# piyanon108/iGate4xSoftphoneDSP

Hardware: AMD Instinct MI355X
Metric: Msamples/s G.711 decode+RMS, 65536ch@8kHz; %HBM roofline at 1/2/4/8 GPU (higher is better)
Workload: dtype u8

## Files before the change

### igate4xsoftphonedsp_amd/csrc/igdsp_device.h

```cpp
#pragma once
#include "igdsp_internal.h"

#include <algorithm>
#include <cstdlib>

namespace igdsp {

__device__ __forceinline__ uint32_t ulaw_abs(uint32_t code)
{
    const uint32_t u = ~code & 0x7Fu;
    return ((((u & 15u) * 2u + 33u) << (u >> 4)) - 33u) << 2;
}

__device__ __forceinline__ uint32_t alaw_abs(uint32_t code)
{
    const uint32_t a = (code ^ 0x55u) & 0x7Fu;
    const uint32_t s = a >> 4, q = a & 15u;
    const uint32_t m = (s == 0u) ? (q * 2u + 1u) : ((q * 2u + 33u) << (s - 1u));
    return m << 3;
}

typedef uint32_t u32x4_t __attribute__((ext_vector_type(4)));
__device__ __forceinline__ uint4 ld_stream(const uint4 *p)
{
// ... 28 lines not shown
__device__ __forceinline__ __amdgpu_buffer_rsrc_t make_rsrc_ranged(const void *base, uint32_t bytes)
{
    return __builtin_amdgcn_make_buffer_rsrc(const_cast<void *>(base), 0, (int)bytes, 0x00020000);
}
__device__ __forceinline__ uint4 buf_ld_stream(__amdgpu_buffer_rsrc_t r, uint32_t voff, uint32_t soff)
{
    const u32x4_t v = __builtin_amdgcn_raw_buffer_load_b128(r, (int)voff, (int)soff, 2);
    return make_uint4(v.x, v.y, v.z, v.w);
}
#ifndef IGDSP_RTS_LOAD_AUX
#define IGDSP_RTS_LOAD_AUX 2
#endif
__device__ __forceinline__ uint4 buf_ld_pieces(__amdgpu_buffer_rsrc_t r, uint32_t voff, uint32_t soff)
{
    const u32x4_t v = __builtin_amdgcn_raw_buffer_load_b128(r, (int)voff, (int)soff, IGDSP_RTS_LOAD_AUX);
    return make_uint4(v.x, v.y, v.z, v.w);
}
__device__ __forceinline__ void buf_st(__amdgpu_buffer_rsrc_t r, uint32_t voff, uint32_t soff, const uint4 v)
{
    u32x4_t t; t.x = v.x; t.y = v.y; t.z = v.z; t.w = v.w;
    __builtin_amdgcn_raw_buffer_store_b128(t, r, (int)voff, (int)soff, 0);
}

#ifndef IGDSP_RECORD_STORE
#define IGDSP_RECORD_STORE 2
#endif
__device__ __forceinline__ void st_record_block(igdsp_frame_stats *base, uint32_t lane, const uint4 v)
{
#if IGDSP_RECORD_STORE == 2
    u32x4_t t; t.x = v.x; t.y = v.y; t.z = v.z; t.w = v.w;
    __builtin_amdgcn_raw_buffer_store_b128(t, make_rsrc(base), (int)(lane * 16u), 0, 16);
#elif IGDSP_RECORD_STORE == 1
    u32x4_t t; t.x = v.x; t.y = v.y; t.z = v.z; t.w = v.w;
    __builtin_nontemporal_store(t, reinterpret_cast<u32x4_t *>(base) + lane);
#else
    st_stream(reinterpret_cast<uint4 *>(base) + lane, v);
#endif
}

__device__ __forceinline__ uint32_t full_scale(bool alaw) { return alaw ? 32256u : 32124u; }

__device__ __forceinline__ uint64_t shfl_xor_u64(uint64_t v, int m)
{
    uint32_t lo = (uint32_t)v, hi = (uint32_t)(v >> 32);
    lo = (uint32_t)__shfl_xor((int)lo, m, 64);
    hi = (uint32_t)__shfl_xor((int)hi, m, 64);
    return ((uint64_t)hi << 32) | lo;
}

__device__ __forceinline__ void agg_commit_block(igdsp_aggregate *agg, uint32_t rank, uint2 *slots, uint32_t nwaves,
                                                 uint64_t sumsq, uint64_t samples, uint32_t frames, uint32_t n_silent,
                                                 uint32_t n_clipped, uint32_t bm_sum, uint32_t peak)
{
    const uint32_t lane = threadIdx.x & 63u, wave = threadIdx.x >> 6;
#pragma unroll
    for (int m = 32; m >= 1; m >>= 1) {
        sumsq += shfl_xor_u64(sumsq, m);
        samples += shfl_xor_u64(samples, m);
        frames += (uint32_t)__shfl_xor((int)frames, m, 64);
        n_silent += (uint32_t)__shfl_xor((int)n_silent, m, 64);
// ... 259 lines not shown
    for (int j = 0; j < kLoadsPerChunk; ++j) {
        const uint32_t p = (uint32_t)j * 64u + lane, f = p / 10u, q = p - f * 10u;
        const uint32_t sh = q == 1u ? 0u : (q == 3u ? 8u : (q == 2u ? 16u : 24u));
        fr5 |= f << (5 * j);
        pm5 |= sh << (5 * j);
    }
}

#ifndef IGDSP_SPREAD_METER
#define IGDSP_SPREAD_METER 0
#endif
__device__ __forceinline__ uint32_t spread_batch(uint32_t b, uint32_t nb)
{
#ifdef IGDSP_NO_SPREAD
    return b;
#endif
    const uint32_t half = (nb + 1u) >> 1;
    return b >= nb ? b : ((b & 1u) ? half + (b >> 1) : (b >> 1));
}

template <int W>
struct BlockQueue { uint32_t next, batch[8], tag[8]; };

template <int W>
__device__ __forceinline__ void bq_init(BlockQueue<W> &q, uint32_t *gq, uint32_t G, uint32_t gb1)
{
    q.next = (uint32_t)W;
    for (int i = 0; i < 8; ++i) q.tag[i] = 0xFFFFFFFFu;
    q.batch[0] = blockIdx.x; q.tag[0] = 0u;
    q.batch[1] = gq ? gb1 + G : blockIdx.x + G; q.tag[1] = 1u;
}

template <int W>
__device__ __forceinline__ uint32_t bq_grab(BlockQueue<W> &q, uint32_t *gq, uint32_t G, uint32_t lane, uint32_t nb)
{
    uint32_t v = 0;
    if (lane == 0) {
        const uint32_t s = atomicAdd(&q.next, 1u);
        const uint32_t j = s / (uint32_t)W, w = s - j * (uint32_t)W;
        if (w == 0u) {
            const uint32_t nb = gq ? atomicAdd(gq, 1u) + G : blockIdx.x + (j + 1u) * G;
            __hip_atomic_store(&q.batch[(j + 1u) & 7u], nb, __ATOMIC_RELAXED, __HIP_MEMORY_SCOPE_WORKGROUP);
            __hip_atomic_store(&q.tag[(j + 1u) & 7u], j + 1u, __ATOMIC_RELEASE, __HIP_MEMORY_SCOPE_WORKGROUP);
        }
        while (__hip_atomic_load(&q.tag[j & 7u], __ATOMIC_ACQUIRE, __HIP_MEMORY_SCOPE_WORKGROUP) != j)
            __builtin_amdgcn_s_sleep(2);
        v = spread_batch(__hip_atomic_load(&q.batch[j & 7u], __ATOMIC_RELAXED, __HIP_MEMORY_SCOPE_WORKGROUP), nb) * (uint32_t)W + w;
    }
    return (uint32_t)__builtin_amdgcn_readfirstlane((int)v);
}

__device__ __forceinline__ void bq_finish(uint32_t *gq, uint32_t G)
{
    if (gq == nullptr) return;
    __syncthreads();
    if (threadIdx.x == 0 && atomicAdd(gq + 1, 1u) == G - 1u) { gq[0] = 0u; gq[1] = 0u; }
}

template <typename T> __device__ __forceinline__ void lds_add(T *p, T v) { __hip_atomic_fetch_add(p, v, __ATOMIC_RELAXED, __HIP_MEMORY_SCOPE_WORKGROUP); }
__device__ __forceinline__ void lds_max(uint32_t *p, uint32_t v) { __hip_atomic_fetch_max(p, v, __ATOMIC_RELAXED, __HIP_MEMORY_SCOPE_WORKGROUP); }
__device__ __forceinline__ void lds_min(uint32_t *p, uint32_t v) { __hip_atomic_fetch_min(p, v, __ATOMIC_RELAXED, __HIP_MEMORY_SCOPE_WORKGROUP); }
__device__ __forceinline__ uint32_t wave_draw(uint32_t *counter, uint32_t lane)
{
    uint32_t v = 0;
// ... 181 lines not shown
```

### igate4xsoftphonedsp_amd/csrc/igdsp_k_meter.hip

```cpp
#include "igdsp_device.h"

namespace igdsp {

__global__ __launch_bounds__(256) void k_meter_wave_per_frame(
    const uint8_t *__restrict__ payload, const uint8_t *__restrict__ codec, const uint16_t *__restrict__ len,
    uint32_t C, uint32_t first_frame, uint32_t n_frames, uint32_t n, igdsp_frame_stats *__restrict__ stats,
    int16_t *__restrict__ pcm, igdsp_aggregate *agg, uint32_t rank)
{
    __shared__ int16_t lut[2][256];
    __shared__ uint2 agg_slots[4 * 4];
    for (uint32_t i = threadIdx.x; i < 512u; i += 256u) {
        const uint32_t code = i & 255u;
        const int ax = (int)((i >> 8) ? alaw_abs(code) : ulaw_abs(code));
        lut[i >> 8][code] = (int16_t)((code & 0x80u) ? ax : -ax);
    }
    __syncthreads();

    const uint32_t lane = threadIdx.x & 63u, wave = threadIdx.x >> 6;
    const bool dword_ok = ((n & 3u) == 0u) && ((reinterpret_cast<uintptr_t>(payload) & 3u) == 0u) &&
                          ((reinterpret_cast<uintptr_t>(pcm) & 7u) == 0u);
    uint64_t a_sumsq = 0, a_samples = 0;
    uint32_t a_frames = 0, a_sil = 0, a_clip = 0, a_bm = 0, a_peak = 0;

    auto load_frame = [&](uint32_t fi) -> uint32_t {
// ... 376 lines not shown
                        u_sil += (uint32_t)__builtin_popcountll(__ballot((fl & IGDSP_FLAG_SILENT) != 0u));
                        u_clip += (uint32_t)__builtin_popcountll(__ballot((fl & IGDSP_FLAG_CLIPPED) != 0u));
                    }
                }
                wave_lds_fence();
            }
            if (done) break;
        }
    }
    if (AGG && agg != nullptr) {
        const bool l0 = lane == 0u;
        agg_commit_block(agg, rank, lds + kLutEntries, (uint32_t)kFatWaves, a_sumsq, l0 ? (uint64_t)u_frames * kFrame : 0ull, l0 ? u_frames : 0u,
                         l0 ? u_sil : 0u, l0 ? u_clip : 0u, a_bm, a_peak);
    }
}

constexpr int kImgMaxPieces = IGDSP_MAX_PAYLOAD * kSuperFrames / 16 / 64;

template <bool AGG, bool RAGGED>
__global__ __launch_bounds__(kImgMaxWaves * 64) void k_meter_image(
    const uint8_t *__restrict__ payload, const uint8_t *__restrict__ codec, const uint16_t *__restrict__ len, uint32_t C,
    uint32_t first_frame, uint32_t n_frames, uint32_t n, igdsp_frame_stats *__restrict__ stats, igdsp_aggregate *agg, uint32_t rank)
{
    __shared__ uint2 lut[kLutEntries];
    extern __shared__ __attribute__((aligned(16))) uint8_t img_smem[];
    const uint32_t n_waves = blockDim.x >> 6;
    fill_lut(lut);
    __syncthreads();
    const uint32_t lane = threadIdx.x & 63u, wave = (uint32_t)__builtin_amdgcn_readfirstlane((int)(threadIdx.x >> 6));
    const uint32_t img_bytes = (uint32_t)kSuperFrames * n;
    uint32_t *img = reinterpret_cast<uint32_t *>(img_smem + (size_t)wave * img_bytes);
    const uint32_t off = (lane & 31u) * 8u;
    const uint32_t D = n >> 2;
    const uint32_t np = (img_bytes / 16u + 63u) >> 6;
    const uint32_t n_items = (n_frames - first_frame + (uint32_t)kSuperFrames - 1u) / (uint32_t)kSuperFrames;
    const uint64_t total_bytes = (uint64_t)n_frames * n;
    const uint8_t *base0 = payload + (uint64_t)first_frame * n;

    uint64_t a_sumsq = 0;
    uint32_t a_samp = 0, a_bm = 0, a_peak = 0;
    uint32_t u_frames = 0, u_sil = 0, u_clip = 0;

    uint4 d[kImgMaxPieces];
    auto avail_of = [&](uint32_t it) {
        const uint64_t b = (uint64_t)first_frame * n + (uint64_t)it * img_bytes;
        return (uint32_t)min((uint64_t)img_bytes, total_bytes - b);
    };
    auto fetch = [&](uint32_t it) {
        const uint8_t *src = base0 + (uint64_t)it * img_bytes;
        const uint32_t avail = avail_of(it);
// ... 81 lines not shown
                    uint32_t w = row[i];
                    const uint32_t nv = min(l - 4u * i, 4u);
                    const uint32_t t = (w & 0x7F7F7F7Fu) | lm;
                    const uint2 e0 = lut_at(lut, t, off, 0x0C0C0400u), e1 = lut_at(lut, t, off, 0x0C0C0500u);
                    const uint2 e2 = lut_at(lut, t, off, 0x0C0C0600u), e3 = lut_at(lut, t, off, 0x0C0C0700u);
                    if (nv == 4u) {
                        part += e0.x + e1.x + e2.x + e3.x;
                        peak = max(max(peak, e0.y), max(e1.y, max(e2.y, e3.y)));
                    } else {
                        part += e0.x + (nv > 1u ? e1.x : 0u) + (nv > 2u ? e2.x : 0u);
                        peak = max(max(peak, e0.y), max(nv > 1u ? e1.y : 0u, nv > 2u ? e2.y : 0u));
                        w &= (1u << (8u * nv)) - 1u;
                    }
                    bsum = __builtin_amdgcn_sad_u8(w, 0u, bsum);
                }
            }
            s += part;
        }
        bool probe = false;
        if (l > 48u) probe = ((row[7] & 0xFFu) == 0xD5u) && (((row[9] >> 16) & 0xFFu) == 0xD5u) && ((row[12] & 0xFFu) == 0xD5u);
        uint32_t bm = 0, fl = 0;
        uint4 rec = make_uint4(0u, 0u, 0u, (uint32_t)IGDSP_FLAG_EMPTY << 24);
        if (l != 0u) rec = pack_stats(s << 4, peak, bsum, l, alaw, probe, bm, fl);
        if (live) st_stream(reinterpret_cast<uint4 *>(stats + fi), rec);
        if (AGG) {
            const bool met = l != 0u;
            if (met) { a_sumsq += s << 4; a_samp += l; a_bm += bm; a_peak = max(a_peak, peak); }
            u_frames += (uint32_t)__builtin_popcountll(__ballot(met));
            u_sil += (uint32_t)__builtin_popcountll(__ballot(met && (fl & IGDSP_FLAG_SILENT) != 0u));
            u_clip += (uint32_t)__builtin_popcountll(__ballot(met && (fl & IGDSP_FLAG_CLIPPED) != 0u));
        }
        wave_lds_fence();
    }
    if (AGG && agg != nullptr) {
        __shared__ uint2 agg_slots[kWavesPerBlock * 4];
        const bool l0 = lane == 0u;
        agg_commit_block(agg, rank, agg_slots, n_waves, a_sumsq, (uint64_t)a_samp, l0 ? u_frames : 0u, l0 ? u_sil : 0u, l0 ? u_clip : 0u, a_bm, a_peak);
    }
}


template <int Q, bool TAIL, bool AGG, bool STORE = false>
__global__ __launch_bounds__((StridedGeom<Q + (TAIL ? 1 : 0), STORE>::kWaves * 64)) void k_meter_strided(
    const uint8_t *__restrict__ payload, const uint8_t *__restrict__ codec, uint32_t C, uint32_t n_frames, uint32_t n,
    igdsp_frame_stats *__restrict__ stats, igdsp_aggregate *agg, uint32_t rank, uint32_t *gqueue, int16_t *__restrict__ pcm = nullptr)
{
    static_assert(Q == 1 || Q >= 4, "the probe bytes 28 / 38 / 48 are taken from pieces 1 / 2 / 3");
    constexpr int QP = Q + (TAIL ? 1 : 0);
    constexpr int kWaves = StridedGeom<QP, STORE>::kWaves;
    constexpr int kRow = QP | 1;
    constexpr int kStrip = kSuperFrames * kRow;
    constexpr int kLutU2 = STORE ? kLutEntries : kLut32Words / 2;
    __shared__ uint2 lds[kLutU2 + kWaves * kStrip + (STORE ? kWaves * 256 : 0)];
    __shared__ BlockQueue<kWaves> bq;
    __shared__ AggBlock aggb;
    uint32_t gb1 = 0;
    if (threadIdx.x == 0 && gqueue != nullptr) gb1 = atomicAdd(gqueue, 1u);
    if (STORE) fill_lut(lds); else fill_lut32(reinterpret_cast<uint32_t *>(lds));
    if (threadIdx.x == 0) { bq_init(bq, gqueue, gridDim.x, gb1); agg_block_init(aggb); }
    __syncthreads();

    const uint32_t lane = threadIdx.x & 63u, wave = (uint32_t)__builtin_amdgcn_readfirstlane((int)(threadIdx.x >> 6));
    uint2 *strip = lds + kLutU2 + wave * kStrip;
    uint8_t *xpose = STORE ? reinterpret_cast<uint8_t *>(lds + kLutU2 + kWaves * kStrip + wave * 256) : nullptr;
    const uint32_t off = (lane & 31u) * (STORE ? 8u : 4u);
    const uint32_t *l32 = reinterpret_cast<const uint32_t *>(lds);
    const uint32_t T = (n - 16u * Q) >> 2;
    constexpr int kPk = (QP + 1) / 2;
    constexpr bool kPoRegs = !STORE || QP <= 11;
    uint32_t pk[kPk];
    uint32_t po[kPoRegs ? QP : 1];
#pragma unroll
    for (int j = 0; j < kPk; ++j) pk[j] = 0;
#pragma unroll
    for (int j = 0; j < QP; ++j) {
        const uint32_t p = (uint32_t)j * 64u + lane, f = p / (uint32_t)QP, q = p - f * (uint32_t)QP;
        const uint32_t sh = q == 1u ? 0u : (q == 3u ? 8u : (q == 2u ? 16u : 24u));
        const bool tp = TAIL && q == (uint32_t)Q;
        pk[j >> 1] |= ((f << 2) | ((tp ? 24u : sh) << 8) | (tp ? 0x2000u : 0u)) << (16 * (j & 1));
        if (kPoRegs) po[j] = f * n + (tp ? n - 16u : 16u * q);
    }
// ... 145 lines not shown
#pragma unroll
                    for (int t = 0; t < 2; ++t)
                        if ((uint32_t)t < T) {
                            const uint32_t w = tws[t];
                            if (STORE) {
                                const uint32_t tt = (w & 0x7F7F7F7Fu) | lm;
                                const uint2 e0 = lut_at(lds, tt, off, 0x0C0C0400u), e1 = lut_at(lds, tt, off, 0x0C0C0500u);
                                const uint2 e2 = lut_at(lds, tt, off, 0x0C0C0600u), e3 = lut_at(lds, tt, off, 0x0C0C0700u);
                                s += (uint64_t)(e0.x + e1.x + e2.x + e3.x);
                                peak = max(max(peak, e0.y), max(e1.y, max(e2.y, e3.y)));
                            } else {
                                const uint32_t ot = off | (lm & 0x80u);
                                const uint32_t q0 = lut32_at(l32, w, ot, 0x0C0C0400u), q1 = lut32_at(l32, w, ot, 0x0C0C0500u);
                                const uint32_t q2 = lut32_at(l32, w, ot, 0x0C0C0600u), q3 = lut32_at(l32, w, ot, 0x0C0C0700u);
                                s += (uint64_t)(q0 + q1 + q2 + q3);
                                tail_m2 = max(tail_m2, max(max(q0, q1), max(q2, q3)));
                            }
                            bsum = __builtin_amdgcn_sad_u8(w, 0u, bsum);
                        }
                    if (!STORE) peak = max(peak, isqrt_m2(tail_m2) << 2);
                }
                const bool probe = (Q >= 4) && (fail >> 31) == 0u;
                uint32_t bm, fl;
                st_stream(reinterpret_cast<uint4 *>(stats + (f0 + lane)), pack_stats(s << 4, peak, bsum, n, my_alaw, probe, bm, fl));
                if (AGG) {
                    a_sumsq += s << 4; a_bm += bm; a_peak = max(a_peak, peak);
                    u_frames += (uint32_t)kSuperFrames;
                    u_sil += (uint32_t)__builtin_popcountll(__ballot((fl & IGDSP_FLAG_SILENT) != 0u));
                    u_clip += (uint32_t)__builtin_popcountll(__ballot((fl & IGDSP_FLAG_CLIPPED) != 0u));
                }
            }
            wave_lds_fence();
            return nxt_pt;
        };
        auto load_item = [&](uint4 (&d)[QP], const uint32_t s) __attribute__((always_inline)) {
            const uint8_t *b0 = payload + (uint64_t)s * item_bytes;
#pragma unroll
            for (int j = 0; j < QP; ++j) d[j] = ld16_dw(b0 + po_of(j));
        };
        if (!kTwoAhead) {
            uint4 d[QP];
            uint32_t sidx = sidx0, cur_pt = fetch_pt(sidx);
            load_item(d, sidx);
            uint32_t s_next = grab();
            for (;;) {
                const bool has_next = s_next < n_super;
                uint32_t s_after;
// ... 88 lines not shown
    for (int d = 0; d < kTinyDepth; ++d) { ids[d] = next_item(); fetch(ids[d], q[d]); }
#endif
    auto step = [&](Item &slot, uint32_t &id) __attribute__((always_inline)) -> bool {
        const uint32_t it = id;
        if (it == 0xFFFFFFFFu) return false;
        const Item x = slot;
        id = next_item();
        fetch(id, slot);
        const bool alaw = x.pt == IGDSP_PT_PCMA;
        const uint32_t oj = off | (alaw ? 0x80u : 0u);
        uint32_t sum = 0, mx = 0, bsum = 0;
        auto dword = [&](uint32_t w) {
            const uint32_t q0 = lut32_at(l32, w, oj, 0x0C0C0400u), q1 = lut32_at(l32, w, oj, 0x0C0C0500u);
            const uint32_t q2 = lut32_at(l32, w, oj, 0x0C0C0600u), q3 = lut32_at(l32, w, oj, 0x0C0C0700u);
            sum = sum + q0 + q1; sum = sum + q2 + q3;
            mx = max(max(mx, q0), q1); mx = max(max(mx, q2), q3);
            bsum = __builtin_amdgcn_sad_u8(w, 0u, bsum);
        };
        dword(x.a.x); dword(x.a.y); dword(x.a.z); dword(x.a.w);
#pragma unroll
        for (int k = 4; k < N4; ++k) dword(x.b[k - 4]);
        const uint32_t peak = isqrt_m2(mx) << 2;
        uint32_t bm, fl;
        st_stream(reinterpret_cast<uint4 *>(stats + ((uint64_t)it * (uint32_t)kSuperFrames + lane)),
                  pack_stats((uint64_t)sum << 4, peak, bsum, n, alaw, false, bm, fl));
        if (AGG) {
            a_sumsq += (uint64_t)sum << 4; a_bm += bm; a_peak = max(a_peak, peak);
            u_frames += (uint32_t)kSuperFrames;
            u_sil += (uint32_t)__builtin_popcountll(__ballot((fl & IGDSP_FLAG_SILENT) != 0u));
            u_clip += (uint32_t)__builtin_popcountll(__ballot((fl & IGDSP_FLAG_CLIPPED) != 0u));
        }
        return true;
    };
    static_assert(kTinyDepth == 4, "the loop below names the four register sets");
    while (step(q[0], ids[0]) && step(q[1], ids[1]) && step(q[2], ids[2]) && step(q[3], ids[3])) {}
    wave_exit(AGG ? agg : nullptr, rank, aggb, (uint32_t)kTinyWaves, lane, gqueue, G, a_sumsq, lane == 0u ? (uint64_t)u_frames * n : 0ull,
              a_bm, a_peak, u_frames, u_sil, u_clip);
}

hipError_t init_device_attributes()
{
    const int lim = 160 * 1024 - 2048 - kLutEntries * 8;
    const void *fns[] = {reinterpret_cast<const void *>(&k_meter_image<true, true>), reinterpret_cast<const void *>(&k_meter_image<false, true>),
                         reinterpret_cast<const void *>(&k_meter_image<true, false>), reinterpret_cast<const void *>(&k_meter_image<false, false>)};
    for (const void *f : fns) {
        const hipError_t e = hipFuncSetAttribute(f, hipFuncAttributeMaxDynamicSharedMemorySize, lim);
        if (e != hipSuccess) return e;
    }
// ... 59 lines not shown
```

### igate4xsoftphonedsp_amd/csrc/igdsp_k_packets.hip

```cpp
#include "igdsp_device.h"
#include "igdsp_rtp.h"

namespace igdsp {

constexpr int kSlotPieces = IGDSP_SLOT_BYTES / 16;
constexpr int kRtpHalfLoads = kSlotPieces * kChunkFrames / 64;
constexpr int kRtpRow = kSlotPieces + 2;
constexpr int kRtpStrip = kSuperFrames * kRtpRow;

template <bool SLOT, bool MIXED = false>
__device__ __forceinline__ void rtp_half(const uint2 *lut, uint2 *strip_half, uint4 (&d)[kRtpHalfLoads],
                                         const uint32_t am, const uint32_t (&fr)[kRtpHalfLoads], const uint32_t (&pm)[kRtpHalfLoads],
                                         const uint32_t off, const uint32_t lane,
                                         const uint8_t *refill_base, const uint32_t (&roff)[kRtpHalfLoads], const uint32_t nrm = 0u)
{
    uint2 e[2][8];
    uint32_t wa[2], wb[2];
    auto issue = [&](int u) {
        const int j = u >> 1, k = u & 1;
        wa[k] = (u & 1) ? d[j].z : d[j].x;
        wb[k] = (u & 1) ? d[j].w : d[j].y;
        const uint32_t lmj = (uint32_t)__builtin_amdgcn_sbfe(am, fr[j], 1) & 0x80808080u;
        const uint32_t ta = (wa[k] & 0x7F7F7F7Fu) | lmj, tb = (wb[k] & 0x7F7F7F7Fu) | lmj;
        e[k][0] = lut_at(lut, ta, off, 0x0C0C0400u); e[k][1] = lut_at(lut, ta, off, 0x0C0C0500u);
        e[k][2] = lut_at(lut, ta, off, 0x0C0C0600u); e[k][3] = lut_at(lut, ta, off, 0x0C0C0700u);
        e[k][4] = lut_at(lut, tb, off, 0x0C0C0400u); e[k][5] = lut_at(lut, tb, off, 0x0C0C0500u);
        e[k][6] = lut_at(lut, tb, off, 0x0C0C0600u); e[k][7] = lut_at(lut, tb, off, 0x0C0C0700u);
// ... 113 lines not shown
    }
}

template <bool AGG, bool SLOT, bool MIXED = false, int WIN = 0>
__global__ __launch_bounds__(kRtpWaves * 64) void k_meter_rtp64(
    const uint8_t *__restrict__ slots, const uint16_t *__restrict__ sizes, const uint8_t *__restrict__ codec, uint32_t C,
    uint32_t n_frames, uint32_t stride, uint32_t hdr, igdsp_frame_stats *__restrict__ stats, igdsp_rtp_info *__restrict__ info,
    igdsp_aggregate *agg, uint32_t rank, uint32_t *gqueue, const uint8_t *__restrict__ radio = nullptr, const WinArgs win = WinArgs{})
{
    static_assert(!(SLOT && MIXED), "slots always hold 20-byte headers");
    if (MIXED) hdr = 12u;
    __shared__ __attribute__((aligned(16))) uint2 lds[kLutEntries + kRtpWaves * kRtpStrip];
    __shared__ BlockQueue<kRtpWaves> bq;
    __shared__ AggBlock aggb;
    __shared__ BlkHoldWindowT<WIN == 2> wst;
    __shared__ uint32_t w_ticket;
    __shared__ uint32_t w_run[WIN == 2 ? kBlkCh : 1], w_alarms[WIN == 2 ? kBlkCh : 1], w_commit[4];
    __shared__ __attribute__((aligned(16))) uint4 w_ring[WIN == 2 ? 4 * kWinRing : 1];
    __shared__ uint32_t w_flag[WIN == 2 ? 4 * kWinRing : 1];
    uint32_t gb1 = 0;
#ifdef IGDSP_BLK_STAMP
    const uint64_t t_stamp0 = wall_clock64();
#endif
    if (threadIdx.x == 0 && gqueue != nullptr) gb1 = atomicAdd(gqueue, 1u);
    igdsp_chan_probe p0 = igdsp_chan_probe{0u, 0u};
    if (WIN == 2 && threadIdx.x < win.gpb * 64u && win.probe != nullptr) p0 = win.probe[blockIdx.x * win.gpb * 64u + threadIdx.x];
    fill_lut(lds);
    if (threadIdx.x == 0) { bq_init(bq, gqueue, gridDim.x, gb1); agg_block_init(aggb); if (WIN == 2) { bq.next = 0u; w_ticket = 0u; } }
    if constexpr (WIN == 2) {
        wst.init(threadIdx.x, blockDim.x);
        if (threadIdx.x < win.gpb * 64u) { w_run[threadIdx.x] = p0.run; w_alarms[threadIdx.x] = p0.alarms; }
        if (threadIdx.x < 4u) w_commit[threadIdx.x] = 0u;
        if (threadIdx.x < 4u * (uint32_t)kWinRing) w_flag[threadIdx.x] = 0u;
    }
    const uint32_t lane = threadIdx.x & 63u, wave = (uint32_t)__builtin_amdgcn_readfirstlane((int)(threadIdx.x >> 6));
    __syncthreads();

    uint2 *strip = lds + kLutEntries + wave * kRtpStrip;
    const uint32_t off = (lane & 31u) * 8u;
    uint32_t pm[kRtpHalfLoads], fr[kRtpHalfLoads];
    uint32_t roff0[kRtpHalfLoads], roff1[kRtpHalfLoads];
#pragma unroll
    for (int j = 0; j < kRtpHalfLoads; ++j) {
        const uint32_t p = (uint32_t)j * 64u + lane;
        const uint32_t f = p / 12u;
        const uint32_t q = p - f * 12u;
        fr[j] = f | ((q < 2u ? q + 1u : 0u) << 8);
        pm[j] = q < 2u ? 0u : probe_mask(q - 2u);
        if (SLOT) {
            roff0[j] = p * 16u;
            roff1[j] = (p + (uint32_t)(kChunkFrames * kSlotPieces)) * 16u;
        } else {
            const uint32_t po = q == 0u ? 0u : (q == 1u ? 4u : hdr + 16u * (q - 2u));
            roff0[j] = f * stride + po;
            roff1[j] = (f + (uint32_t)kChunkFrames) * stride + po;
        }
    }
    const uint32_t G = gridDim.x;
    const uint32_t n_super = n_frames / kSuperFrames;
    const uint64_t super_bytes = (uint64_t)kSuperFrames * (SLOT ? (uint32_t)IGDSP_SLOT_BYTES : stride);
    uint64_t a_sumsq = 0;
    uint32_t a_samp = 0, a_bm = 0, a_peak = 0;
    uint32_t u_frames = 0, u_sil = 0, u_clip = 0;

    auto fetch_radio = [&](uint32_t sidx) { return MIXED ? (uint32_t)radio[(sidx * (uint32_t)kSuperFrames + lane) % C] : 0u; };
    auto offsets = [&](uint64_t rm, uint32_t (&o0)[kRtpHalfLoads], uint32_t (&o1)[kRtpHalfLoads]) {
#pragma unroll
        for (int j = 0; j < kRtpHalfLoads; ++j) {
            const uint32_t f = fr[j] & 31u, b0 = (uint32_t)(rm >> f) & 1u, b1 = (uint32_t)(rm >> (f + 32u)) & 1u;
            o0[j] = roff0[j] + (fr[j] < 256u ? 8u * b0 : 0u);
            o1[j] = roff1[j] + (fr[j] < 256u ? 8u * b1 : 0u);
        }
    };
    auto ld = [&](const uint8_t *b, uint32_t o) { return SLOT ? ld_stream(reinterpret_cast<const uint4 *>(b + o)) : ld16_dw(b + o); };
    auto fetch_pt = [&](uint32_t sidx) { return (uint32_t)codec[(sidx * (uint32_t)kSuperFrames + lane) % C]; };
    const uint32_t n_batches = IGDSP_SPREAD_METER ? (n_super + (uint32_t)kRtpWaves - 1u) / (uint32_t)kRtpWaves : 0u;
    uint32_t w_next = 0, w_left = 0, w_seg = 0, w_unit = wave * G + blockIdx.x;
    const uint32_t nw = WIN ? (uint32_t)(blockDim.x >> 6) : (uint32_t)kRtpWaves;
    const uint32_t w_units = win.n_groups * win.n_seg, w_stride = G * nw;
    const uint32_t b_items = win.F * win.gpb, b_first = blockIdx.x * win.gpb;
    auto grab = [&]() -> uint32_t {
        if (!WIN) return bq_grab(bq, gqueue, G, lane, n_batches);
        if (WIN == 2) {
            const uint32_t v = wave_draw(&bq.next, lane);
            return v < b_items ? v : 0xFFFFFFFFu;
        }
#ifdef IGDSP_WIN_ASC
        { const uint32_t id = w_unit; w_unit += w_stride; return id < n_super ? id : 0xFFFFFFFFu; }
#endif
        if (w_left == 0u) {
            if (w_unit >= w_units) return 0xFFFFFFFFu;
            w_seg = w_unit / win.n_groups;
            const uint32_t f_lo = (uint32_t)(((uint64_t)win.F * w_seg) / win.n_seg);
            w_left = (uint32_t)(((uint64_t)win.F * (w_seg + 1u)) / win.n_seg) - f_lo;
            w_next = f_lo * win.n_groups + (w_unit - w_seg * win.n_groups);
            w_unit += w_stride;
        }
        const uint32_t id = w_next | (w_seg << 27) | (w_left == 1u ? 0x80000000u : 0u);
        w_next += win.n_groups;
        w_left -= 1u;
        return id;
    };
    auto id_ok = [&](uint32_t id) { return WIN ? id != 0xFFFFFFFFu : id < n_super; };
    auto id_sidx = [&](uint32_t id) { return WIN == 2 ? (id >> win.gsh) * win.n_groups + b_first + (id & (win.gpb - 1u)) : (WIN ? (id & 0x07FFFFFFu) : id); };
    uint64_t w_sumsq = 0;
    uint32_t w_cnt = 0, w_lsum = 0, w_samp = 0, w_pm = 0, w_min = 255u, w_sc = 0;
    uint32_t r_trail = 0, r_lead = 0, r_hits = 0;

    igdsp_chan_hold e_hold = igdsp_chan_hold{};
    uint32_t e_ticket = 0xFFFFFFFFu;
    bool e_open = false;
    auto end_prefetch = [&]() {
        e_ticket = wave_draw(&w_ticket, lane);
        if (e_ticket < win.gpb) {
            const uint32_t c = (b_first + e_ticket) * 64u + lane;
            e_hold = win.hold[c];
            e_open = win.gate == nullptr || win.gate[c] != 0;
        }
    };
    uint32_t id_cur = WIN ? grab() : spread_batch(blockIdx.x, n_batches) * (uint32_t)kRtpWaves + wave;
    uint32_t sidx = id_sidx(id_cur);
    if (id_ok(id_cur)) {
        uint4 X[kRtpHalfLoads], Y[kRtpHalfLoads];
        uint32_t cur_pt = fetch_pt(sidx);
        uint32_t cur_radio = fetch_radio(sidx);
        {
            const uint8_t *b0 = slots + (uint64_t)sidx * super_bytes;
            if (MIXED) {
                uint32_t o0[kRtpHalfLoads], o1[kRtpHalfLoads];
                offsets(__ballot(cur_radio != 0u), o0, o1);
#pragma unroll
                for (int j = 0; j < kRtpHalfLoads; ++j) X[j] = ld(b0, o0[j]);
#pragma unroll
                for (int j = 0; j < kRtpHalfLoads; ++j) Y[j] = ld(b0, o1[j]);
            } else {
#pragma unroll
                for (int j = 0; j < kRtpHalfLoads; ++j) X[j] = ld(b0, roff0[j]);
#pragma unroll
                for (int j = 0; j < kRtpHalfLoads; ++j) Y[j] = ld(b0, roff1[j]);
            }
        }
        uint32_t s_next = grab();
        for (;;) {
            const bool has_next = id_ok(s_next);
            if (WIN == 2 && !has_next) end_prefetch();
            const uint32_t s_load = has_next ? id_sidx(s_next) : 0u;
            const uint32_t f0 = sidx * kSuperFrames;
            const bool my_alaw = cur_pt == IGDSP_PT_PCMA;
            const uint64_t amask = __ballot(my_alaw);
// ... 40 lines not shown
                uint32_t hf = (((w0 >> 6) & 3u) == 2u ? IGDSP_RTP_V2 : 0u) | ((w0 & 0x10u) ? IGDSP_RTP_X : 0u) |
                              ((w0 & 0x8000u) ? IGDSP_RTP_MARKER : 0u);
                uint32_t ed = 0, plen = 0;
                if (size < hbytes) hf = IGDSP_RTP_RUNT;
                else {
                    plen = size - hbytes;
                    if (hbytes == 20u) {
                        if (pt == 8u || pt == 0u || pt == 18u || pt == 123u) ed = __builtin_bswap32(h.w);
                        if ((w0 & 0x10u) && h.z == 0x01006701u) hf |= IGDSP_RTP_ED137_OK;
                    }
                    if (pt == 123u) hf |= IGDSP_RTP_KEEPALIVE;
                    if (plen > (uint32_t)kFrame) hf |= IGDSP_RTP_OVERSIZE;
                    else if ((pt == 0u || pt == 8u) && plen > 0u) hf |= IGDSP_RTP_METERED;
                }
                const bool pt_ok = pt == cur_pt && (pt == 0u || pt == 8u);
                const bool whole = size == full && pt_ok;
                const bool shortp = pt_ok && size > hbytes && size < full;
                const bool metered = whole || shortp;
                const uint32_t fi = f0 + lane;
                if (info != nullptr) {
                    uint2 rec;
                    rec.x = ed;
                    rec.y = (size < hbytes ? 0u : plen) | ((size >= 2u ? pt : 0u) << 16) | (hf << 24);
                    *reinterpret_cast<uint2 *>(info + fi) = rec;
                }
                uint32_t bm = 0, fl = 0;
                uint4 rec = make_uint4(0u, 0u, 0u, (uint32_t)IGDSP_FLAG_EMPTY << 24);
                if (whole) rec = pack_stats160(s, peak, bsum, my_alaw, (fail >> 31) == 0u, bm, fl);
                if (__ballot(shortp) != 0ull) {
                    if (shortp) {
                        const uint8_t *pp = slots + (uint64_t)sidx * super_bytes + lane * (SLOT ? (uint32_t)IGDSP_SLOT_BYTES : stride) +
                                            (SLOT ? (uint32_t)IGDSP_SLOT_PAYLOAD_OFFSET : hbytes);
                        bool pr;
                        meter_short(lds, off, pp, plen, my_alaw, s, peak, bsum, pr);
                        rec = pack_stats(s << 4, peak, bsum, plen, my_alaw, pr, bm, fl);
                    }
                }
                if (!WIN || stats != nullptr) st_stream(reinterpret_cast<uint4 *>(stats + fi), rec);
                if (AGG) {
                    if (metered) { a_sumsq += s << 4; a_samp += whole ? (uint32_t)kFrame : plen; a_bm += bm; a_peak = max(a_peak, peak); }
                    u_frames += (uint32_t)__builtin_popcountll(__ballot(metered));
                    u_sil += (uint32_t)__builtin_popcountll(__ballot(metered && (fl & IGDSP_FLAG_SILENT) != 0u));
                    u_clip += (uint32_t)__builtin_popcountll(__ballot(metered && (fl & IGDSP_FLAG_CLIPPED) != 0u));
                }
                if constexpr (WIN == 2) {
                    win_blk_item(win, id_cur, lane, whole ? (uint32_t)kFrame : plen, metered, ed, s << 4, peak, bm, fl, c_seen, c_run, c_al,
                                 wst, w_commit, w_flag, w_ring, w_run, w_alarms);
                } else if (WIN) {
#ifndef IGDSP_WIN_NOBOOK
                    const uint32_t l = whole ? (uint32_t)kFrame : plen;
                    const bool valid = metered && l > 48u, pr = valid && (fl & IGDSP_FLAG_PROBE_D5) != 0u, npr = valid && !pr;
                    const uint32_t nt = r_trail + (pr ? 1u : 0u);
                    r_hits += (pr && (r_lead >> 31) != 0u && nt == win.alarm) ? 1u : 0u;
                    r_lead = (npr && (r_lead >> 31) == 0u) ? (r_trail | 0x80000000u) : r_lead;
                    r_trail = npr ? 0u : nt;
                    const bool fold = metered && (win.gate_mask == 0u || (ed & win.gate_mask) != 0u);
                    w_sumsq += fold ? (s << 4) : 0ull;
                    w_cnt += fold ? 1u : 0u; w_lsum += fold ? bm : 0u; w_samp += fold ? l : 0u;
                    w_pm = __builtin_bit_cast(uint32_t, __builtin_elementwise_max(__builtin_bit_cast(v2u16_t, w_pm), __builtin_bit_cast(v2u16_t, fold ? (peak | (bm << 16)) : 0u)));
                    w_min = min(w_min, fold ? bm : 255u);
                    w_sc += fold ? (((fl & IGDSP_FLAG_SILENT) ? 1u : 0u) + ((fl & IGDSP_FLAG_CLIPPED) ? 0x10000u : 0u)) : 0u;
// ... 264 lines not shown
```

Measured before the change: 6.010 million.

## Add per-kernel record store policies, early RTP loads, paired info stores, LUT-once

Moves the per-frame stats record stores in the image, strided and RTP kernels onto selectable cache policies, with the write-through buffer store as the default for several paths. The RTP kernel now issues its first superframe loads before LUT setup and the barrier, and uses a static second batch in the block queue so those early loads need not wait on a global atomic. RTP info records are merged in lane pairs through DPP into 16-byte stores. LUT filling switches to a fill-once variant. The aim is to hide startup latency and reduce store-side cache pollution and transaction count, at the cost of more compile-time variants and a changed work-queue schedule.

Result: no change. 6.009 million (-0.0%).

```diff
diff --git a/igate4xsoftphonedsp_amd/csrc/igdsp_device.h b/igate4xsoftphonedsp_amd/csrc/igdsp_device.h
--- a/igate4xsoftphonedsp_amd/csrc/igdsp_device.h
+++ b/igate4xsoftphonedsp_amd/csrc/igdsp_device.h
@@ -74,20 +74,55 @@
     __builtin_amdgcn_raw_buffer_store_b128(t, r, (int)voff, (int)soff, 0);
 }
 
+template <int POLICY, typename Index>
+__device__ __forceinline__ void st_record_block_as(igdsp_frame_stats *stats, Index f0, uint32_t lane, const uint4 v)
+{
+    static_assert(POLICY == 0 || POLICY == 1 || POLICY == 2, "0 cached, 1 nontemporal, 2 write-through");
+    if constexpr (POLICY == 2) {
+        u32x4_t t; t.x = v.x; t.y = v.y; t.z = v.z; t.w = v.w;
+        __builtin_amdgcn_raw_buffer_store_b128(t, make_rsrc(stats + f0), (int)(lane * 16u), 0, 16);
+    } else if constexpr (POLICY == 1) {
+        u32x4_t t; t.x = v.x; t.y = v.y; t.z = v.z; t.w = v.w;
+        __builtin_nontemporal_store(t, reinterpret_cast<u32x4_t *>(stats + (f0 + lane)));
+    } else {
+        st_stream(reinterpret_cast<uint4 *>(stats + (f0 + lane)), v);
+    }
+}
 #ifndef IGDSP_RECORD_STORE
 #define IGDSP_RECORD_STORE 2
 #endif
+#ifndef IGDSP_RTP_RECORD_STORE
+#define IGDSP_RTP_RECORD_STORE 2
+#endif
+#ifndef IGDSP_RTP_PACKED_RECORD_STORE
+#define IGDSP_RTP_PACKED_RECORD_STORE 0
+#endif
+#ifndef IGDSP_RTP_WIN_RECORD_STORE
+#define IGDSP_RTP_WIN_RECORD_STORE 0
+#endif
+#ifndef IGDSP_STRIDED_RECORD_STORE
+#define IGDSP_STRIDED_RECORD_STORE 2
+#endif
+#ifndef IGDSP_STRIDED_PCM_RECORD_STORE
+#define IGDSP_STRIDED_PCM_RECORD_STORE 0
+#endif
+#ifndef IGDSP_TINY_RECORD_STORE
+#define IGDSP_TINY_RECORD_STORE 0
+#endif
+#ifndef IGDSP_IMAGE_RECORD_STORE
+#define IGDSP_IMAGE_RECORD_STORE 2
+#endif
 __device__ __forceinline__ void st_record_block(igdsp_frame_stats *base, uint32_t lane, const uint4 v)
 {
-#if IGDSP_RECORD_STORE == 2
-    u32x4_t t; t.x = v.x; t.y = v.y; t.z = v.z; t.w = v.w;
-    __builtin_amdgcn_raw_buffer_store_b128(t, make_rsrc(base), (int)(lane * 16u), 0, 16);
-#elif IGDSP_RECORD_STORE == 1
-    u32x4_t t; t.x = v.x; t.y = v.y; t.z = v.z; t.w = v.w;
-    __builtin_nontemporal_store(t, reinterpret_cast<u32x4_t *>(base) + lane);
-#else
-    st_stream(reinterpret_cast<uint4 *>(base) + lane, v);
-#endif
+    st_record_block_as<IGDSP_RECORD_STORE>(base, 0u, lane, v);
+}
+
+__device__ __forceinline__ void st_info_pairs(igdsp_rtp_info *base, uint32_t lane, const uint2 v)
+{
+    const uint32_t nx = (uint32_t)__builtin_amdgcn_update_dpp(0, (int)v.x, 0xF5, 0xF, 0xF, false);
+    const uint32_t ny = (uint32_t)__builtin_amdgcn_update_dpp(0, (int)v.y, 0xF5, 0xF, 0xF, false);
+    u32x4_t t; t.x = v.x; t.y = v.y; t.z = nx; t.w = ny;
+    if ((lane & 1u) == 0u) __builtin_amdgcn_raw_buffer_store_b128(t, make_rsrc(base), (int)(lane * 8u), 0, 16);
 }
 
 __device__ __forceinline__ uint32_t full_scale(bool alaw) { return alaw ? 32256u : 32124u; }
@@ -393,16 +428,16 @@
 template <int W>
 struct BlockQueue { uint32_t next, batch[8], tag[8]; };
 
-template <int W>
+template <int W, bool STATIC2 = false>
 __device__ __forceinline__ void bq_init(BlockQueue<W> &q, uint32_t *gq, uint32_t G, uint32_t gb1)
 {
     q.next = (uint32_t)W;
     for (int i = 0; i < 8; ++i) q.tag[i] = 0xFFFFFFFFu;
     q.batch[0] = blockIdx.x; q.tag[0] = 0u;
-    q.batch[1] = gq ? gb1 + G : blockIdx.x + G; q.tag[1] = 1u;
-}
-
-template <int W>
+    q.batch[1] = (gq && !STATIC2) ? gb1 + G : blockIdx.x + G; q.tag[1] = 1u;
+}
+
+template <int W, bool STATIC2 = false>
 __device__ __forceinline__ uint32_t bq_grab(BlockQueue<W> &q, uint32_t *gq, uint32_t G, uint32_t lane, uint32_t nb)
 {
     uint32_t v = 0;
@@ -410,7 +445,7 @@
         const uint32_t s = atomicAdd(&q.next, 1u);
         const uint32_t j = s / (uint32_t)W, w = s - j * (uint32_t)W;
         if (w == 0u) {
-            const uint32_t nb = gq ? atomicAdd(gq, 1u) + G : blockIdx.x + (j + 1u) * G;
+            const uint32_t nb = gq ? atomicAdd(gq, 1u) + (STATIC2 ? 2u : 1u) * G : blockIdx.x + (j + 1u) * G;
             __hip_atomic_store(&q.batch[(j + 1u) & 7u], nb, __ATOMIC_RELAXED, __HIP_MEMORY_SCOPE_WORKGROUP);
             __hip_atomic_store(&q.tag[(j + 1u) & 7u], j + 1u, __ATOMIC_RELEASE, __HIP_MEMORY_SCOPE_WORKGROUP);
         }
diff --git a/igate4xsoftphonedsp_amd/csrc/igdsp_k_meter.hip b/igate4xsoftphonedsp_amd/csrc/igdsp_k_meter.hip
--- a/igate4xsoftphonedsp_amd/csrc/igdsp_k_meter.hip
+++ b/igate4xsoftphonedsp_amd/csrc/igdsp_k_meter.hip
@@ -422,10 +422,10 @@
     const uint8_t *__restrict__ payload, const uint8_t *__restrict__ codec, const uint16_t *__restrict__ len, uint32_t C,
     uint32_t first_frame, uint32_t n_frames, uint32_t n, igdsp_frame_stats *__restrict__ stats, igdsp_aggregate *agg, uint32_t rank)
 {
-    __shared__ uint2 lut[kLutEntries];
+    __shared__ __attribute__((aligned(16))) uint2 lut[kLutEntries];
     extern __shared__ __attribute__((aligned(16))) uint8_t img_smem[];
     const uint32_t n_waves = blockDim.x >> 6;
-    fill_lut(lut);
+    fill_lut_once(lut);
     __syncthreads();
     const uint32_t lane = threadIdx.x & 63u, wave = (uint32_t)__builtin_amdgcn_readfirstlane((int)(threadIdx.x >> 6));
     const uint32_t img_bytes = (uint32_t)kSuperFrames * n;
@@ -553,7 +553,7 @@
         uint32_t bm = 0, fl = 0;
         uint4 rec = make_uint4(0u, 0u, 0u, (uint32_t)IGDSP_FLAG_EMPTY << 24);
         if (l != 0u) rec = pack_stats(s << 4, peak, bsum, l, alaw, probe, bm, fl);
-        if (live) st_stream(reinterpret_cast<uint4 *>(stats + fi), rec);
+        if (live) st_record_block_as<IGDSP_IMAGE_RECORD_STORE>(stats, first_frame + item * (uint32_t)kSuperFrames, lane, rec);
         if (AGG) {
             const bool met = l != 0u;
             if (met) { a_sumsq += s << 4; a_samp += l; a_bm += bm; a_peak = max(a_peak, peak); }
@@ -582,12 +582,12 @@
     constexpr int kRow = QP | 1;
     constexpr int kStrip = kSuperFrames * kRow;
     constexpr int kLutU2 = STORE ? kLutEntries : kLut32Words / 2;
-    __shared__ uint2 lds[kLutU2 + kWaves * kStrip + (STORE ? kWaves * 256 : 0)];
+    __shared__ __attribute__((aligned(16))) uint2 lds[kLutU2 + kWaves * kStrip + (STORE ? kWaves * 256 : 0)];
     __shared__ BlockQueue<kWaves> bq;
     __shared__ AggBlock aggb;
     uint32_t gb1 = 0;
     if (threadIdx.x == 0 && gqueue != nullptr) gb1 = atomicAdd(gqueue, 1u);
-    if (STORE) fill_lut(lds); else fill_lut32(reinterpret_cast<uint32_t *>(lds));
+    if (STORE) fill_lut_once(lds); else fill_lut32(reinterpret_cast<uint32_t *>(lds));
     if (threadIdx.x == 0) { bq_init(bq, gqueue, gridDim.x, gb1); agg_block_init(aggb); }
     __syncthreads();
 
@@ -779,7 +779,7 @@
                 }
                 const bool probe = (Q >= 4) && (fail >> 31) == 0u;
                 uint32_t bm, fl;
-                st_stream(reinterpret_cast<uint4 *>(stats + (f0 + lane)), pack_stats(s << 4, peak, bsum, n, my_alaw, probe, bm, fl));
+                st_record_block_as<(STORE ? IGDSP_STRIDED_PCM_RECORD_STORE : IGDSP_STRIDED_RECORD_STORE)>(stats, f0, lane, pack_stats(s << 4, peak, bsum, n, my_alaw, probe, bm, fl));
                 if (AGG) {
                     a_sumsq += s << 4; a_bm += bm; a_peak = max(a_peak, peak);
                     u_frames += (uint32_t)kSuperFrames;
@@ -914,8 +914,8 @@
         for (int k = 4; k < N4; ++k) dword(x.b[k - 4]);
         const uint32_t peak = isqrt_m2(mx) << 2;
         uint32_t bm, fl;
-        st_stream(reinterpret_cast<uint4 *>(stats + ((uint64_t)it * (uint32_t)kSuperFrames + lane)),
-                  pack_stats((uint64_t)sum << 4, peak, bsum, n, alaw, false, bm, fl));
+        st_record_block_as<IGDSP_TINY_RECORD_STORE>(stats, (uint64_t)it * (uint32_t)kSuperFrames, lane,
+                                                    pack_stats((uint64_t)sum << 4, peak, bsum, n, alaw, false, bm, fl));
         if (AGG) {
             a_sumsq += (uint64_t)sum << 4; a_bm += bm; a_peak = max(a_peak, peak);
             u_frames += (uint32_t)kSuperFrames;
diff --git a/igate4xsoftphonedsp_amd/csrc/igdsp_k_packets.hip b/igate4xsoftphonedsp_amd/csrc/igdsp_k_packets.hip
--- a/igate4xsoftphonedsp_amd/csrc/igdsp_k_packets.hip
+++ b/igate4xsoftphonedsp_amd/csrc/igdsp_k_packets.hip
@@ -3,6 +3,15 @@
 
 namespace igdsp {
 
+#ifndef IGDSP_RTP_EARLY_LOADS
+#define IGDSP_RTP_EARLY_LOADS 1
+#endif
+#ifndef IGDSP_RTP_LUT_ONCE
+#define IGDSP_RTP_LUT_ONCE 1
+#endif
+#ifndef IGDSP_RTP_INFO_STORE
+#define IGDSP_RTP_INFO_STORE 2
+#endif
 constexpr int kSlotPieces = IGDSP_SLOT_BYTES / 16;
 constexpr int kRtpHalfLoads = kSlotPieces * kChunkFrames / 64;
 constexpr int kRtpRow = kSlotPieces + 2;
@@ -162,65 +171,89 @@
 #ifdef IGDSP_BLK_STAMP
     const uint64_t t_stamp0 = wall_clock64();
 #endif
-    if (threadIdx.x == 0 && gqueue != nullptr) gb1 = atomicAdd(gqueue, 1u);
+    constexpr bool kEarly = WIN == 0 && !MIXED && (IGDSP_RTP_EARLY_LOADS == 2 || (IGDSP_RTP_EARLY_LOADS == 1 && SLOT));
+    constexpr int kRecordStore = WIN ? IGDSP_RTP_WIN_RECORD_STORE : (SLOT ? IGDSP_RTP_RECORD_STORE : IGDSP_RTP_PACKED_RECORD_STORE);
+    constexpr bool kInfoPairs = IGDSP_RTP_INFO_STORE == 2 && kRecordStore == 2;
+    if (!kEarly && threadIdx.x == 0 && gqueue != nullptr) gb1 = atomicAdd(gqueue, 1u);
+    const uint32_t lane = threadIdx.x & 63u, wave = (uint32_t)__builtin_amdgcn_readfirstlane((int)(threadIdx.x >> 6));
+    uint2 *strip = lds + kLutEntries + wave * kRtpStrip;
+    const uint32_t off = (lane & 31u) * 8u;
+    uint32_t pm[kRtpHalfLoads], fr[kRtpHalfLoads];
+    uint32_t roff0[kRtpHalfLoads], roff1[kRtpHalfLoads];
+    auto piece_consts = [&]() {
+#pragma unroll
+        for (int j = 0; j < kRtpHalfLoads; ++j) {
+            const uint32_t p = (uint32_t)j * 64u + lane;
+            const uint32_t f = p / 12u;
+            const uint32_t q = p - f * 12u;
+            fr[j] = f | ((q < 2u ? q + 1u : 0u) << 8);
+            pm[j] = q < 2u ? 0u : probe_mask(q - 2u);
+            if (SLOT) {
+                roff0[j] = p * 16u;
+                roff1[j] = (p + (uint32_t)(kChunkFrames * kSlotPieces)) * 16u;
+            } else {
+                const uint32_t po = q == 0u ? 0u : (q == 1u ? 4u : hdr + 16u * (q - 2u));
+                roff0[j] = f * stride + po;
+                roff1[j] = (f + (uint32_t)kChunkFrames) * stride + po;
+            }
+        }
+    };
+    if (kEarly) piece_consts();
+    const uint32_t G = gridDim.x;
+    const uint32_t n_super = n_frames / kSuperFrames;
+    const uint64_t super_bytes = (uint64_t)kSuperFrames * (SLOT ? (uint32_t)IGDSP_SLOT_BYTES : stride);
+    auto fetch_radio = [&](uint32_t sidx) { return MIXED ? (uint32_t)radio[(sidx * (uint32_t)kSuperFrames + lane) % C] : 0u; };
+    auto offsets = [&](uint64_t rm, uint32_t (&o0)[kRtpHalfLoads], uint32_t (&o1)[kRtpHalfLoads]) {
+#pragma unroll
+        for (int j = 0; j < kRtpHalfLoads; ++j) {
+            const uint32_t f = fr[j] & 31u, b0 = (uint32_t)(rm >> f) & 1u, b1 = (uint32_t)(rm >> (f + 32u)) & 1u;
+            o0[j] = roff0[j] + (fr[j] < 256u ? 8u * b0 : 0u);
+            o1[j] = roff1[j] + (fr[j] < 256u ? 8u * b1 : 0u);
+        }
+    };
+    auto ld = [&](const uint8_t *b, uint32_t o) { return SLOT ? ld_stream(reinterpret_cast<const uint4 *>(b + o)) : ld16_dw(b + o); };
+    auto fetch_pt = [&](uint32_t sidx) { return (uint32_t)codec[(sidx * (uint32_t)kSuperFrames + lane) % C]; };
+    const uint32_t n_batches = IGDSP_SPREAD_METER ? (n_super + (uint32_t)kRtpWaves - 1u) / (uint32_t)kRtpWaves : 0u;
+    const bool info_pairs = (reinterpret_cast<uintptr_t>(info) & 15u) == 0u;
+    uint4 X[kRtpHalfLoads], Y[kRtpHalfLoads];
+    uint32_t id_cur = WIN ? 0u : spread_batch(blockIdx.x, n_batches) * (uint32_t)kRtpWaves + wave;
+    uint32_t cur_pt = 0;
+    if constexpr (kEarly) {
+        const uint32_t s0 = id_cur < n_super ? id_cur : 0u;
+        cur_pt = fetch_pt(s0);
+        const uint8_t *b0 = slots + (uint64_t)s0 * super_bytes;
+#pragma unroll
+        for (int j = 0; j < kRtpHalfLoads; ++j) X[j] = ld(b0, roff0[j]);
+#pragma unroll
+        for (int j = 0; j < kRtpHalfLoads; ++j) Y[j] = ld(b0, roff1[j]);
+    }
     igdsp_chan_probe p0 = igdsp_chan_probe{0u, 0u};
     if (WIN == 2 && threadIdx.x < win.gpb * 64u && win.probe != nullptr) p0 = win.probe[blockIdx.x * win.gpb * 64u + threadIdx.x];
+#if IGDSP_RTP_LUT_ONCE
+    fill_lut_once(lds);
+#else
     fill_lut(lds);
-    if (threadIdx.x == 0) { bq_init(bq, gqueue, gridDim.x, gb1); agg_block_init(aggb); if (WIN == 2) { bq.next = 0u; w_ticket = 0u; } }
+#endif
+    if (threadIdx.x == 0) { bq_init<kRtpWaves, kEarly>(bq, gqueue, gridDim.x, gb1); agg_block_init(aggb); if (WIN == 2) { bq.next = 0u; w_ticket = 0u; } }
     if constexpr (WIN == 2) {
         wst.init(threadIdx.x, blockDim.x);
         if (threadIdx.x < win.gpb * 64u) { w_run[threadIdx.x] = p0.run; w_alarms[threadIdx.x] = p0.alarms; }
         if (threadIdx.x < 4u) w_commit[threadIdx.x] = 0u;
         if (threadIdx.x < 4u * (uint32_t)kWinRing) w_flag[threadIdx.x] = 0u;
     }
-    const uint32_t lane = threadIdx.x & 63u, wave = (uint32_t)__builtin_amdgcn_readfirstlane((int)(threadIdx.x >> 6));
     __syncthreads();
-
-    uint2 *strip = lds + kLutEntries + wave * kRtpStrip;
-    const uint32_t off = (lane & 31u) * 8u;
-    uint32_t pm[kRtpHalfLoads], fr[kRtpHalfLoads];
-    uint32_t roff0[kRtpHalfLoads], roff1[kRtpHalfLoads];
-#pragma unroll
-    for (int j = 0; j < kRtpHalfLoads; ++j) {
-        const uint32_t p = (uint32_t)j * 64u + lane;
-        const uint32_t f = p / 12u;
-        const uint32_t q = p - f * 12u;
-        fr[j] = f | ((q < 2u ? q + 1u : 0u) << 8);
-        pm[j] = q < 2u ? 0u : probe_mask(q - 2u);
-        if (SLOT) {
-            roff0[j] = p * 16u;
-            roff1[j] = (p + (uint32_t)(kChunkFrames * kSlotPieces)) * 16u;
-        } else {
-            const uint32_t po = q == 0u ? 0u : (q == 1u ? 4u : hdr + 16u * (q - 2u));
-            roff0[j] = f * stride + po;
-            roff1[j] = (f + (uint32_t)kChunkFrames) * stride + po;
-        }
-    }
-    const uint32_t G = gridDim.x;
-    const uint32_t n_super = n_frames / kSuperFrames;
-    const uint64_t super_bytes = (uint64_t)kSuperFrames * (SLOT ? (uint32_t)IGDSP_SLOT_BYTES : stride);
+    if (!kEarly) piece_consts();
+
     uint64_t a_sumsq = 0;
     uint32_t a_samp = 0, a_bm = 0, a_peak = 0;
     uint32_t u_frames = 0, u_sil = 0, u_clip = 0;
 
-    auto fetch_radio = [&](uint32_t sidx) { return MIXED ? (uint32_t)radio[(sidx * (uint32_t)kSuperFrames + lane) % C] : 0u; };
-    auto offsets = [&](uint64_t rm, uint32_t (&o0)[kRtpHalfLoads], uint32_t (&o1)[kRtpHalfLoads]) {
-#pragma unroll
-        for (int j = 0; j < kRtpHalfLoads; ++j) {
-            const uint32_t f = fr[j] & 31u, b0 = (uint32_t)(rm >> f) & 1u, b1 = (uint32_t)(rm >> (f + 32u)) & 1u;
-            o0[j] = roff0[j] + (fr[j] < 256u ? 8u * b0 : 0u);
-            o1[j] = roff1[j] + (fr[j] < 256u ? 8u * b1 : 0u);
-        }
-    };
-    auto ld = [&](const uint8_t *b, uint32_t o) { return SLOT ? ld_stream(reinterpret_cast<const uint4 *>(b + o)) : ld16_dw(b + o); };
-    auto fetch_pt = [&](uint32_t sidx) { return (uint32_t)codec[(sidx * (uint32_t)kSuperFrames + lane) % C]; };
-    const uint32_t n_batches = IGDSP_SPREAD_METER ? (n_super + (uint32_t)kRtpWaves - 1u) / (uint32_t)kRtpWaves : 0u;
     uint32_t w_next = 0, w_left = 0, w_seg = 0, w_unit = wave * G + blockIdx.x;
     const uint32_t nw = WIN ? (uint32_t)(blockDim.x >> 6) : (uint32_t)kRtpWaves;
     const uint32_t w_units = win.n_groups * win.n_seg, w_stride = G * nw;
     const uint32_t b_items = win.F * win.gpb, b_first = blockIdx.x * win.gpb;
     auto grab = [&]() -> uint32_t {
-        if (!WIN) return bq_grab(bq, gqueue, G, lane, n_batches);
+        if (!WIN) return bq_grab<kRtpWaves, kEarly>(bq, gqueue, G, lane, n_batches);
         if (WIN == 2) {
             const uint32_t v = wave_draw(&bq.next, lane);
             return v < b_items ? v : 0xFFFFFFFFu;
@@ -258,13 +291,12 @@
             e_open = win.gate == nullptr || win.gate[c] != 0;
         }
     };
-    uint32_t id_cur = WIN ? grab() : spread_batch(blockIdx.x, n_batches) * (uint32_t)kRtpWaves + wave;
+    if (WIN) id_cur = grab();
     uint32_t sidx = id_sidx(id_cur);
     if (id_ok(id_cur)) {
-        uint4 X[kRtpHalfLoads], Y[kRtpHalfLoads];
-        uint32_t cur_pt = fetch_pt(sidx);
+        if (!kEarly) cur_pt = fetch_pt(sidx);
         uint32_t cur_radio = fetch_radio(sidx);
-        {
+        if (!kEarly) {
             const uint8_t *b0 = slots + (uint64_t)sidx * super_bytes;
             if (MIXED) {
                 uint32_t o0[kRtpHalfLoads], o1[kRtpHalfLoads];
@@ -351,7 +383,8 @@
                     uint2 rec;
                     rec.x = ed;
                     rec.y = (size < hbytes ? 0u : plen) | ((size >= 2u ? pt : 0u) << 16) | (hf << 24);
-                    *reinterpret_cast<uint2 *>(info + fi) = rec;
+                    if (kInfoPairs && info_pairs) st_info_pairs(info + f0, lane, rec);
+                    else *reinterpret_cast<uint2 *>(info + fi) = rec;
                 }
                 uint32_t bm = 0, fl = 0;
                 uint4 rec = make_uint4(0u, 0u, 0u, (uint32_t)IGDSP_FLAG_EMPTY << 24);
@@ -365,7 +398,7 @@
                         rec = pack_stats(s << 4, peak, bsum, plen, my_alaw, pr, bm, fl);
                     }
                 }
-                if (!WIN || stats != nullptr) st_stream(reinterpret_cast<uint4 *>(stats + fi), rec);
+                if (!WIN || stats != nullptr) st_record_block_as<kRecordStore>(stats, f0, lane, rec);
                 if (AGG) {
                     if (metered) { a_sumsq += s << 4; a_samp += whole ? (uint32_t)kFrame : plen; a_bm += bm; a_peak = max(a_peak, peak); }
                     u_frames += (uint32_t)__builtin_popcountll(__ballot(metered));
```
